# gooey-audio/libgooey

Hardware: NVIDIA B200
Metric: voice-samples/sec (higher is better)
Workload: dtype f32

## Files before the change

### libgooey_b200/csrc/dsp.cuh

```cuda
#pragma once
#include "gmath.cuh"

#ifdef __CUDACC__
#define G_HD __host__ __device__ __forceinline__
#define G_D __device__ __forceinline__
#else
#define G_HD inline
#define G_D inline
#endif

namespace gd {

constexpr float PI_F = 3.14159265358979323846f;

G_HD float clampf(float x, float lo, float hi) { return x < lo ? lo : (x > hi ? hi : x); }
G_HD float denorm(float n, float mn, float mx) { return mn + clampf(n, 0.0f, 1.0f) * (mx - mn); }
G_HD float fract(float x) { return x - truncf(x); }

G_HD float u64_to_f32(uint64_t h) {
#ifdef __CUDA_ARCH__
  return __ull2float_rn(h);
#else
  return (float)h;
#endif
// ... 186 lines not shown
  const uint64_t b = 8ull << 56;
  v3 ^= b; G_SIPROUND v0 ^= b;
  v2 ^= 0xff; G_SIPROUND G_SIPROUND G_SIPROUND
  return v0 ^ v1 ^ v2 ^ v3;
}
G_HD float hash_noise(uint64_t idx) {
  float n = u64_to_f32(siphash13_u64(idx)) / 18446744073709551616.0f;
  return n * 2.0f - 1.0f;
}

constexpr int INV_SQ_N = 1024;
#ifdef __CUDACC__
__constant__ float c_inv_sq[INV_SQ_N];
#endif
template <bool FAST = false> G_HD float osc_sine(float idx, float freq, float sr) {
  const float two_pi = 2.0f * PI_F;
  const float x = idx * freq * two_pi / sr;
  if (FAST) return gm::g_sinf_fast(x);
  return gm::g_sinf(x);
}
G_HD float osc_sine_fast(float idx, float freq, float sr, float rcp_sr) {
  const float two_pi = 2.0f * PI_F;
  return gm::g_sinf_fast(gm::g_div_by(idx * freq * two_pi, sr, rcp_sr));
}
G_HD float inv_sq_odd(int i, float fi) {
#ifdef __CUDA_ARCH__
  return c_inv_sq[i >> 1];
#else
  return 1.0f / (fi * fi);
#endif
}
template <bool FAST> G_HD float tri_partial(float idx, float hf, float sr, float rcp_sr) {
  return FAST ? osc_sine_fast(idx, hf, sr, rcp_sr) : osc_sine<false>(idx, hf, sr);
}
template <bool FAST = false> G_HD float osc_triangle(float idx, float freq, float sr) {
  float output = 0.0f;
  const float nyquist = sr / 2.0f;
  const float rcp_sr = 1.0f / sr;
  const float rcp_nyq = 2.0f * rcp_sr;
  const float lim = 0.7f * nyquist;
  float q = nyquist / freq;
  int max_h = !(q == q) ? 0 : (q >= 2147483648.0f ? 2147483647 : (q <= -2147483648.0f ? (-2147483647 - 1) : (int)q));
  const int cap = (freq > 0.0f && sr > 0.0f) ? (max_h < 2 * INV_SQ_N - 1 ? max_h : 2 * INV_SQ_N - 1) : 0;
  int n1 = 0;
  if (cap >= 1) {
    n1 = ((int)fminf(q * 0.7f, (float)cap) + 1) >> 1;
    while (n1 > 0 && freq * (float)(2 * n1 - 1) > lim) n1--;
    while (2 * n1 + 1 <= cap && !(freq * (float)(2 * n1 + 1) > lim)) n1++;
  }
#ifdef __CUDA_ARCH__
#pragma unroll 4
#endif
  for (int h = 0; h < n1; h++) {
    const int i = 2 * h + 1;
    const float fi = (float)i;
    output += inv_sq_odd(i, fi) * tri_partial<FAST>(idx, freq * fi, sr, rcp_sr);
  }
  int i = 2 * n1 + 1;
  for (; i <= cap; i += 2) {
    const float fi = (float)i;
    const float hf = freq * fi;
    if (hf > nyquist) return output;
    const float ratio = gm::g_div_by(hf, nyquist, rcp_nyq);
    const float t = (ratio - 0.75f) / 0.25f;
    const float taper = ratio > 0.75f ? 1.0f - t * t : 1.0f;
    output += inv_sq_odd(i, fi) * taper * tri_partial<FAST>(idx, hf, sr, rcp_sr);
  }
  for (; i <= max_h; i += 2) {
    float fi = (float)i;
    if (freq * fi > nyquist) break;
    float gain = 1.0f / (fi * fi);
    float hf = freq * fi;
    float taper = 1.0f;
    if (hf > 0.7f * nyquist) {
      float ratio = hf / nyquist;
      if (ratio > 0.75f) { float t = (ratio - 0.75f) / 0.25f; taper = 1.0f - t * t; }
    }
    output += gain * taper * tri_partial<FAST>(idx, hf, sr, rcp_sr);
  }
  return output;
}

constexpr uint64_t XS_SEED = 0x123456789abcdef0ull;
G_HD uint64_t xorshift64s_next(uint64_t& s) {
  uint64_t x = s;
  x ^= x >> 12; x ^= x << 25; x ^= x >> 27;
  s = x;
  return x * 0x2545f4914f6cdd1dull;
}
struct Pink { uint64_t rng; float f0, f1, f2; };
struct PinkCoef { float p0, p1, p2, g0, g1, g2; };
G_HD void pink_reset(Pink& p) { p.rng = XS_SEED; p.f0 = p.f1 = p.f2 = 0.0f; }
G_HD PinkCoef pink_coefs(float sr) {
  const float RP[3] = {0.99765f, 0.96300f, 0.57000f};
  const float RG[3] = {0.0990460f, 0.2965164f, 1.0526913f};
  sr = fmaxf(sr, 1.0f);
  float ratio = 44100.0f / sr;
  float po[3], ga[3];
  for (int i = 0; i < 3; i++) {
    po[i] = gm::g_powf(RP[i], ratio);
    ga[i] = RG[i] * sqrtf((1.0f - po[i] * po[i]) / (1.0f - RP[i] * RP[i]));
  }
  return {po[0], po[1], po[2], ga[0], ga[1], ga[2]};
}
G_HD float pink_tick(Pink& p, const PinkCoef& c) {
  uint64_t h = xorshift64s_next(p.rng);
#ifdef __CUDA_ARCH__
  float w = gm::g_div_by((float)(uint32_t)(h >> 40), 16777215.0f, 0x1.000002p-24f);
#else
  float w = (float)(uint32_t)(h >> 40) / 16777215.0f;
#endif
  w = w * 2.0f - 1.0f;
  p.f0 = c.p0 * p.f0 + c.g0 * w;
  p.f1 = c.p1 * p.f1 + c.g1 * w;
  p.f2 = c.p2 * p.f2 + c.g2 * w;
  float s = 0.0f + p.f0;
  s += p.f1;
  s += p.f2;
  return (s + w * 0.1848f) * 0.11f;
}

struct Tpt { float cutoff, res, g, r, h, ic1, ic2; };
G_HD void tpt_update(Tpt& f, float sr) {
  float cutoff = clampf(f.cutoff, 20.0f, sr * 0.45f);
  float q = fmaxf(f.res, 0.5f);
  float g = gm::g_tanf(PI_F * cutoff / sr);
  float r = 1.0f / q;
  f.g = g; f.r = r; f.h = 1.0f / (1.0f + r * g + g * g);
}
G_HD void tpt_init(Tpt& f, float sr, float cutoff, float res) {
  f.cutoff = clampf(cutoff, 20.0f, 20000.0f); f.res = fmaxf(res, 0.5f); f.ic1 = f.ic2 = 0.0f; tpt_update(f, sr);
}
G_HD void tpt_set(Tpt& f, float sr, float cutoff, float res) {
  float nc = clampf(cutoff, 20.0f, sr * 0.45f);
  float nr = fmaxf(res, 0.5f);
  if (fabsf(nc - f.cutoff) > 0.001f || fabsf(nr - f.res) > 0.001f) { f.cutoff = nc; f.res = nr; tpt_update(f, sr); }
}
G_HD void tpt_process(Tpt& f, float in, float& lo, float& bd, float& hi) {
  float v1 = (f.g * (in - f.ic2) + f.ic1) * f.h;
  float v2 = f.ic2 + f.g * v1;
  f.ic1 = 2.0f * v1 - f.ic1;
  f.ic2 = 2.0f * v2 - f.ic2;
  lo = v2; bd = v1; hi = in - (f.r * v1 + v2);
}
G_HD float svf_pick(float lo, float bd, float hi, uint32_t type) {
  return type == 0 ? lo : (type == 2 ? hi : (type == 3 ? lo + hi : bd));
}
G_HD void rlp_update(Tpt& f, float sr) {
  float s = fmaxf(sr, 1.0f);
  float cutoff = clampf(f.cutoff, 20.0f, s * 0.45f);
  float q = clampf(f.res, 0.5f, 10.0f);
  f.g = gm::g_tanf(PI_F * cutoff / s);
  f.r = 1.0f / q;
  f.h = 1.0f / (1.0f + f.r * f.g + f.g * f.g);
}
G_HD void rlp_init(Tpt& f, float sr, float cutoff, float res) {
  f.cutoff = clampf(cutoff, 20.0f, 20000.0f); f.res = clampf(res, 0.5f, 10.0f); f.ic1 = f.ic2 = 0.0f; rlp_update(f, sr);
}
G_HD void rlp_set(Tpt& f, float sr, float cutoff, float res) {
  cutoff = clampf(cutoff, 20.0f, 20000.0f);
  res = clampf(res, 0.5f, 10.0f);
  if (fabsf(cutoff - f.cutoff) > 0.001f || fabsf(res - f.res) > 0.001f) { f.cutoff = cutoff; f.res = res; rlp_update(f, sr); }
}
G_HD float rlp_process(Tpt& f, float in) {
  float v1 = (f.g * (in - f.ic2) + f.ic1) * f.h;
  float v2 = f.ic2 + f.g * v1;
  f.ic1 = 2.0f * v1 - f.ic1;
  f.ic2 = 2.0f * v2 - f.ic2;
  return fabsf(v2) < 1e-15f ? 0.0f : v2;
// ... 214 lines not shown
```

### libgooey_b200/csrc/wave.cuh

```cuda
#pragma once
#include "kernels.cuh"

namespace gd { namespace wave {

__device__ __forceinline__ float shup(float v, int d) { return __shfl_up_sync(0xffffffffu, v, d); }
__device__ __forceinline__ float shl(float v, int n) { return __shfl_sync(0xffffffffu, v, n); }
__device__ __forceinline__ bool gall(bool p) { return __all_sync(0xffffffffu, p); }
__device__ __forceinline__ unsigned gballot(bool p) { return __ballot_sync(0xffffffffu, p); }
__device__ __forceinline__ void gsync() { __syncwarp(); }

struct Geo1 { float m[5]; float ap; };
struct Geo2 { float a; float m[5]; float ap; };

__device__ __forceinline__ Geo1 make_geo1(float a, int lane) {
  Geo1 g; float p = a, ap = 1.0f; const int e = lane + 1;
#pragma unroll
  for (int i = 0; i < 5; i++) { g.m[i] = lane >= (1 << i) ? p : 0.0f; if (e & (1 << i)) ap *= p; p *= p; }
  if (e & 32) ap *= p;
  g.ap = ap;
  return g;
}
__device__ __forceinline__ Geo2 make_geo2(float a, int lane) {
  Geo2 g; g.a = a; float p = a * a, ap = 1.0f;
#pragma unroll
  for (int i = 0; i < 5; i++) { g.m[i] = lane >= (1 << i) ? p : 0.0f; if (lane & (1 << i)) ap *= p; p *= p; }
  g.ap = ap;
  return g;
}
__device__ __forceinline__ float scan1(float b, const Geo1& g, float y_prev) {
#pragma unroll
  for (int i = 0; i < 5; i++) { float t = shup(b, 1 << i); b = __fmaf_rn(g.m[i], t, b); }
  return __fmaf_rn(g.ap, y_prev, b);
}
__device__ __forceinline__ void scan2(float& b0, float& b1, const Geo2& g, float y_prev, int lane) {
  float B = __fmaf_rn(g.a, b0, b1);
#pragma unroll
  for (int i = 0; i < 5; i++) { float t = shup(B, 1 << i); B = __fmaf_rn(g.m[i], t, B); }
  float yp = shup(B, 1);
  if (lane == 0) yp = 0.0f;
  yp = __fmaf_rn(g.ap, y_prev, yp);
  b0 = __fmaf_rn(g.a, yp, b0);
  b1 = __fmaf_rn(g.a, b0, b1);
}
__device__ __forceinline__ float prev_lane(float v, float carry, int lane) { float t = shup(v, 1); return lane == 0 ? carry : t; }

enum { GT_HB = 0, GT_CLICK = 8, GT_DC = 9, GT_PINK = 10, GT_RING = 13, GT_N1 = 14 };
struct GeoTables {
  float g1[GT_N1][6][32];
  float g2[8][7][32];
};
__device__ __forceinline__ void geo_tables_init(GeoTables& T, const RateCtx& rc, int tid, int nthreads) {
  for (int idx = tid; idx < GT_N1 * 32; idx += nthreads) {
    const int i = idx >> 5, lane = idx & 31;
    float ratio;
    if (i < 8) ratio = -c_hb[i];
    else if (i == GT_CLICK) ratio = 1.0f - rc.click_alpha;
    else if (i == GT_DC) ratio = 0.995f;
    else if (i == GT_PINK) ratio = rc.pink.p0;
    else if (i == GT_PINK + 1) ratio = rc.pink.p1;
    else if (i == GT_PINK + 2) ratio = rc.pink.p2;
    else ratio = 0.999f;
    const Geo1 a = make_geo1(ratio, lane);
#pragma unroll
    for (int k = 0; k < 5; k++) T.g1[i][k][lane] = a.m[k];
    T.g1[i][5][lane] = a.ap;
    if (i < 8) {
      const Geo2 b = make_geo2(ratio, lane);
#pragma unroll
      for (int k = 0; k < 5; k++) T.g2[i][1 + k][lane] = b.m[k];
      T.g2[i][0][lane] = b.a; T.g2[i][6][lane] = b.ap;
    }
  }
}
__device__ __forceinline__ Geo1 load_geo1(const GeoTables& T, int i, int lane) {
  Geo1 g;
#pragma unroll
  for (int k = 0; k < 5; k++) g.m[k] = T.g1[i][k][lane];
  g.ap = T.g1[i][5][lane];
  return g;
}
__device__ __forceinline__ Geo2 load_geo2(const GeoTables& T, int i, int lane) {
  Geo2 g; g.a = T.g2[i][0][lane];
#pragma unroll
  for (int k = 0; k < 5; k++) g.m[k] = T.g2[i][1 + k][lane];
  g.ap = T.g2[i][6][lane];
  return g;
}

__device__ __forceinline__ float ap_sec1(float x, float c, const Geo1& g, float& xs, float& ys, int lane, int last) {
  const float xp = prev_lane(x, xs, lane);
  const float y = scan1(__fmaf_rn(c, x, xp), g, ys);
  xs = shl(x, last); ys = shl(y, last);
  return y;
}
__device__ __forceinline__ void ap_sec2(float& x0, float& x1, float c, const Geo2& g, float& xs, float& ys, int lane, int last) {
  const float xp = prev_lane(x1, xs, lane);
  float b0 = __fmaf_rn(c, x0, xp), b1 = __fmaf_rn(c, x1, x0);
  const float nx = shl(x1, last);
  scan2(b0, b1, g, ys, lane);
  xs = nx; ys = shl(b1, last);
  x0 = b0; x1 = b1;
}
__device__ __forceinline__ void hb_run1(Hb8& s, float& p0, float& p1, const GeoTables& T, int lane, int last) {
#pragma unroll
  for (int i = 0; i < 8; i += 2) {
    p0 = ap_sec1(p0, c_hb[i], load_geo1(T, i, lane), s.x[i], s.y[i], lane, last);
    p1 = ap_sec1(p1, c_hb[i + 1], load_geo1(T, i + 1, lane), s.x[i + 1], s.y[i + 1], lane, last);
  }
}
__device__ __forceinline__ void hb_run2(Hb8& s, float& a0, float& a1, float& b0, float& b1, const GeoTables& T, int lane, int last) {
#pragma unroll
  for (int i = 0; i < 8; i += 2) {
    ap_sec2(a0, a1, c_hb[i], load_geo2(T, i, lane), s.x[i], s.y[i], lane, last);
    ap_sec2(b0, b1, c_hb[i + 1], load_geo2(T, i + 1, lane), s.x[i + 1], s.y[i + 1], lane, last);
  }
}
template <class F> __device__ __forceinline__ float os_scan(Oversamp& o, float in, F f, const GeoTables& T, int lane, int last) {
  if (o.mode == 0) return f(in);
  float s0 = in, s1 = in;
  hb_run1(o.outer_up, s0, s1, T, lane, last);
  if (o.mode == 2) {
    float a = f(s1), b = f(s0);
    hb_run1(o.outer_down, a, b, T, lane, last);
    return 0.5f * (a + b);
  }
  float i00 = s0, i01 = s1, i10 = s0, i11 = s1;
  hb_run2(o.inner_up, i00, i01, i10, i11, T, lane, last);
  float a0 = f(i10), a1 = f(i11), b0 = f(i00), b1 = f(i01);
  hb_run2(o.inner_down, a0, a1, b0, b1, T, lane, last);
  const float d0 = 0.5f * (a0 + b0), d1 = 0.5f * (a1 + b1);
  float a = d1, b = d0;
  hb_run1(o.outer_down, a, b, T, lane, last);
  return 0.5f * (a + b);
}

struct Lin2 {
  float P[5][4];
  float L[4][32];
};
__device__ __forceinline__ void mat_mul(const float* a, const float* b, float* c) {
  c[0] = a[0] * b[0] + a[1] * b[2]; c[1] = a[0] * b[1] + a[1] * b[3];
  c[2] = a[2] * b[0] + a[3] * b[2]; c[3] = a[2] * b[1] + a[3] * b[3];
}
__device__ __forceinline__ void lin2_init(Lin2& S, float m0, float m1, float m2, float m3, int lane) {
  float p[4] = {m0, m1, m2, m3}, acc[4] = {1.0f, 0.0f, 0.0f, 1.0f}, t[4];
  const int e = lane + 1;
#pragma unroll
  for (int i = 0; i < 5; i++) {
    if (lane == 0) { S.P[i][0] = p[0]; S.P[i][1] = p[1]; S.P[i][2] = p[2]; S.P[i][3] = p[3]; }
    if (e & (1 << i)) { mat_mul(p, acc, t); acc[0] = t[0]; acc[1] = t[1]; acc[2] = t[2]; acc[3] = t[3]; }
    mat_mul(p, p, t); p[0] = t[0]; p[1] = t[1]; p[2] = t[2]; p[3] = t[3];
  }
  if (e & 32) { mat_mul(p, acc, t); acc[0] = t[0]; acc[1] = t[1]; acc[2] = t[2]; acc[3] = t[3]; }
  S.L[0][lane] = acc[0]; S.L[1][lane] = acc[1]; S.L[2][lane] = acc[2]; S.L[3][lane] = acc[3];
  gsync();
}
__device__ __forceinline__ void lin2_scan(const Lin2& S, float& f0, float& f1, float s0p, float s1p, int lane) {
#pragma unroll
  for (int i = 0; i < 5; i++) {
    const float t0 = shup(f0, 1 << i), t1 = shup(f1, 1 << i);
    if (lane >= (1 << i)) {
      f0 = __fmaf_rn(S.P[i][0], t0, __fmaf_rn(S.P[i][1], t1, f0));
      f1 = __fmaf_rn(S.P[i][2], t0, __fmaf_rn(S.P[i][3], t1, f1));
    }
  }
  f0 = __fmaf_rn(S.L[0][lane], s0p, __fmaf_rn(S.L[1][lane], s1p, f0));
  f1 = __fmaf_rn(S.L[2][lane], s0p, __fmaf_rn(S.L[3][lane], s1p, f1));
}

struct WaveScratch { Lin2 lin[3]; float stash[8][32]; };


__device__ __forceinline__ float w_tanh(float x) {
  const float ax = fabsf(x);
  const float e = __expf(2.0f * ax);
  const float t = 1.0f - __fdividef(2.0f, e + 1.0f);
  return copysignf(t, x);
}
__device__ __forceinline__ float w_gain_comp(FbShaper& w, float env) {
  const float reference = fmaxf(env, 0.05f);
  const float driven = fmaxf(fabsf(w_tanh(reference * w.drive)), 1e-6f);
  const float comp_no_fb = w_tanh(reference) / driven;
  const float makeup = fbws_makeup(w);
  const float taming = 1.0f / (1.0f + comp_no_fb * w.feedback * 0.25f);
  return fminf(comp_no_fb * taming * makeup, 3.0f);
}
__device__ __forceinline__ float wrap01(float x) { return x < 1.0f ? x : (x < 2.0f ? x - 1.0f : fmodf(x, 1.0f)); }

struct TptLin { float in0, in1; };
__device__ __forceinline__ TptLin tpt_lin_init(Lin2& S, const Tpt& f, int lane) {
  const float g = f.g, h = f.h, gh = g * h, g2h = g * gh;
  lin2_init(S, 2.0f * h - 1.0f, -2.0f * gh, 2.0f * gh, 1.0f - 2.0f * g2h, lane);
  TptLin t; t.in0 = 2.0f * gh; t.in1 = 2.0f * g2h;
  return t;
}
__device__ __forceinline__ void tpt_scan(const Lin2& S, const TptLin& t, Tpt& f, float in, float& ic1_pre, float& ic2_pre, int lane, int last) {
  float s0 = t.in0 * in, s1 = t.in1 * in;
  lin2_scan(S, s0, s1, f.ic1, f.ic2, lane);
  ic1_pre = prev_lane(s0, f.ic1, lane); ic2_pre = prev_lane(s1, f.ic2, lane);
  f.ic1 = shl(s0, last); f.ic2 = shl(s1, last);
}
__device__ __forceinline__ void biquad_lin_init(Lin2& S, const Biquad& b, int lane) { lin2_init(S, -b.a1, -b.a2, 1.0f, 0.0f, lane); }
__device__ __forceinline__ float biquad_scan(const Lin2& S, Biquad& b, float x, int lane, int last) {
  const float xm1 = prev_lane(x, b.x1, lane);
  float xm2 = shup(x, 2);
  xm2 = lane == 0 ? b.x2 : (lane == 1 ? b.x1 : xm2);
  float f0 = b.b0 * x + b.b1 * xm1 + b.b2 * xm2, f1 = 0.0f;
  lin2_scan(S, f0, f1, b.y1, b.y2, lane);
  const float nx1 = shl(x, last), nx2 = shl(xm1, last);
  const float ny1 = shl(f0, last), ny2 = shl(f1, last);
  b.x1 = nx1; b.x2 = nx2; b.y1 = ny1; b.y2 = ny2;
  return fabsf(f0) < 1e-15f ? 0.0f : f0;
}

#define LANE_VAL(v, n) shl((v), (n))
#define STASH_PUT(slot, v) (sc.stash[slot][lane] = (v))
#define STASH_GET(slot, n) (sc.stash[slot][n])

struct KickW {
  using V = KickV;
  struct Span2 { bool noise, shaper, serial; };
  static __device__ __forceinline__ int active_end(const KickV::Run& r) { return r.j_act; }
  static __device__ __forceinline__ void span_setup(KickAud& a, const KickV::Run& r, Span2& w, WaveScratch&, const RateCtx& rc, int) {
    w.noise = r.d.noise_amount > 0.001f;
    a.ws.drive = r.d.drive; a.ws.feedback = r.d.feedback;
    fbws_set_cutoff(a.ws, rc.sr, r.d.fb_cutoff);
    w.shaper = !(a.ws.mix <= 0.0001f || a.ws.drive <= 1.0f);
    w.serial = w.shaper && a.ws.feedback != 0.0f;
    if (w.noise) rlp_set(a.noise_lp, rc.sr, r.d.noise_cut, r.d.noise_res);
  }
  static __device__ __forceinline__ float block(KickAud& a, const KickV::Run& r, const Span2& w, WaveScratch& sc, const GeoTables& T,
                                                const float* p, int, int& nl, const RateCtx& rc, int lane) {
    const int last = nl - 1;
    const float p1 = p[0], raw_click = p[1], ne = p[2], amp = p[3];
    float hp_l = 0.0f, fn_l = 0.0f;
    gsync(); STASH_PUT(0, raw_click); gsync();
#pragma unroll 4
    for (int n = 0; n < nl; n++) {
      const float raw = STASH_GET(0, n);
      const float hp = raw - a.click_hp;
      a.click_hp += rc.click_alpha * hp;
      float fn = 0.0f;
      if (w.noise) fn = rlp_process(a.noise_lp, pink_tick(a.pink, rc.pink));
      if (n == lane) { hp_l = hp; fn_l = fn; }
    }
    const float filt_click = hp_l * (1.0f + 4.0f * 0.1f);
    const float noise_out = w.noise ? fn_l * ne * r.d.noise_amount * 0.5f : 0.0f;
    const float total = p1 + filt_click + noise_out;
    float od = total;
    const bool finite = gall(isfinite(total));
    if (w.serial || (w.shaper && !finite)) {
#pragma unroll 4
      for (int n = 0; n < nl; n++) {
        const float y = fbws_process(a.ws, LANE_VAL(total, n));
        if (n == lane) od = y;
      }
    } else if (w.shaper) {
      FbShaper& ws = a.ws;
      const float fb_in = ws.drive * total + ws.feedback * ws.last_out;
      const float shaped = os_scan(ws.os, fb_in, [](float x) { return w_tanh(x); }, T, lane, last);
      const float rect_l = fabsf(total);
      float env_l = 0.0f;
      gsync(); STASH_PUT(1, rect_l); gsync();
#pragma unroll 4
      for (int n = 0; n < nl; n++) {
        const float rect = STASH_GET(1, n);
        const float coeff = rect > ws.env ? ws.env_att : ws.env_rel;
        ws.env += (1.0f - coeff) * (rect - ws.env);
        if (fabsf(ws.env) < 1e-15f) ws.env = 0.0f;
        if (n == lane) env_l = ws.env;
      }
      const float comp = w_gain_comp(ws, env_l);
      const float compensated = shaped * comp;
      float out_l = 0.0f;
      gsync(); STASH_PUT(2, compensated); gsync();
#pragma unroll 4
      for (int n = 0; n < nl; n++) {
        const float c = STASH_GET(2, n);
        const float out = c - ws.dc_x1 + 0.995f * ws.dc_y1;
        ws.dc_x1 = c;
        ws.dc_y1 = fabsf(out) < 1e-15f ? 0.0f : out;
        ws.filter_state += ws.filter_coeff * (out - ws.filter_state);
        if (fabsf(ws.filter_state) < 1e-15f) ws.filter_state = 0.0f;
        if (n == lane) out_l = out;
      }
      ws.last_out = ws.filter_state;
      od = total * (1.0f - ws.mix) + out_l * ws.mix;
    }
    return od * amp * r.d.va * r.d.volume;
  }
};

struct SnareW {
  using V = SnareV;
  struct Span2 { float comp; bool shaper; };
  static __device__ __forceinline__ int active_end(const SnareV::Run& r) { return r.j_act; }
  static __device__ __forceinline__ void span_setup(SnareAud& a, const SnareV::Run& r, Span2& w, WaveScratch&, const RateCtx& rc, int) {
    chamb_set(a.filt, rc.sr, r.d.cutoff, r.d.res);
    a.ws.drive = r.d.drive;
    w.shaper = !(a.ws.mix <= 0.0001f || a.ws.drive <= 1.0f);
    w.comp = w.shaper ? gm::g_tanhf(0.5f) / gm::g_tanhf(0.5f * a.ws.drive) : 1.0f;
  }
  static __device__ __forceinline__ float block(SnareAud& a, const SnareV::Run& r, const Span2& w, WaveScratch& sc, const GeoTables& T,
                                                const float* p, int, int& nl, const RateCtx&, int lane) {
    const int last = nl - 1;
    const float tonal_out = p[0], raw_noise = p[1], cne = p[2], crack_out = p[3], amp = p[4];
    float low_l = 0.0f, band_l = 0.0f, high_l = 0.0f;
    {
      const float f = a.filt.f, q = a.filt.q;
      float low = a.filt.low, band = a.filt.band;
      gsync(); STASH_PUT(0, raw_noise); gsync();
#pragma unroll 4
      for (int n = 0; n < nl; n++) {
        const float in = STASH_GET(0, n);
        float high = 0.0f;
#pragma unroll
        for (int i = 0; i < 2; i++) { low = low + f * band; high = in - low - q * band; band = f * high + band; }
        if (n == lane) { low_l = low; band_l = band; high_l = high; }
      }
      a.filt.low = low; a.filt.band = band;
    }
    const float filtered = svf_pick(low_l, band_l, high_l, r.d.filter_type);
    const float noise_out = filtered * cne * r.d.noise_mix;
    const float total = tonal_out + noise_out + crack_out;
    float od = total;
    const bool finite = gall(isfinite(total));
    if (!finite) {
#pragma unroll 4
      for (int n = 0; n < nl; n++) {
        const float y = ws_process(a.ws, LANE_VAL(total, n));
        if (n == lane) od = y;
      }
    } else if (w.shaper) {
      const float d = a.ws.drive, comp = w.comp;
      const float sat = os_scan(a.ws.os, total, [d, comp](float x) { return w_tanh(x * d) * comp; }, T, lane, last);
      od = total * (1.0f - a.ws.mix) + sat * a.ws.mix;
    }
    return od * amp * r.d.va * r.d.volume;
  }
};

struct HatW {
  using V = HatV;
  struct Span2 { TptLin svf; };
  static __device__ __forceinline__ int active_end(const HatV::Run&) { return 0x7fffffff; }
  static __device__ __forceinline__ void span_setup(HatAud& a, const HatV::Run& r, Span2& w, WaveScratch& sc, const RateCtx& rc, int lane) {
    hp_set(a.hp1, rc.sr, r.d.pitch_hz, 1.0f);
    biquad_lin_init(sc.lin[0], a.hp1, lane);
    if (r.d.db24) { hp_set(a.hp2, rc.sr, r.d.pitch_hz, 1.0f); biquad_lin_init(sc.lin[1], a.hp2, lane); }
    tpt_set(a.svf, rc.sr, r.d.tone_hz, 0.5f);
    w.svf = tpt_lin_init(sc.lin[2], a.svf, lane);
  }
  static __device__ __forceinline__ float block(HatAud& a, const HatV::Run& r, const Span2& w, WaveScratch& sc, const GeoTables&,
                                                const float* p, int j, int& nl, const RateCtx& rc, int lane) {
    const float sr = rc.sr;
    const float env_l = (j + lane) < r.j_env ? p[0] : r.env_final;
    float es_l = 0.0f;
    int nv = nl;
    gsync(); STASH_PUT(0, env_l); gsync();
    if (j + nl <= r.j_env) {
#pragma unroll 4
      for (int n = 0; n < nl; n++) {
        const float e = STASH_GET(0, n);
        if (e >= a.env_smooth) a.env_smooth = e; else a.env_smooth += rc.asym_down * (e - a.env_smooth);
        if (n == lane) es_l = a.env_smooth;
      }
    } else {
#pragma unroll 4
      for (int n = 0; n < nl; n++) {
        const float e = STASH_GET(0, n);
        if (e >= a.env_smooth) a.env_smooth = e; else a.env_smooth += rc.asym_down * (e - a.env_smooth);
        if (n == lane) es_l = a.env_smooth;
        if ((j + n) >= r.j_env && a.env_smooth < 1e-4f) { nv = n + 1; a.active = 0; break; }
      }
    }
    nl = nv;
    float noise = 0.0f, mph = 0.0f, nph = 0.0f;
    const float inc_mod = fmaxf(r.d.pitch_hz * 0.1f, 0.0f) / sr, inc_main = fmaxf(r.d.pitch_hz, 0.0f) / sr;
    const bool small_inc = inc_main < 1.0f && a.mod_phase < 1.0f && a.main_phase < 1.0f;
    if (!r.d.pink_on && small_inc) {
      uint64_t st_l = 0;
#pragma unroll 4
      for (int n = 0; n < nv; n++) {
        uint64_t x = a.white;
        x ^= x >> 12; x ^= x << 25; x ^= x >> 27;
        a.white = x;
        float pm = a.mod_phase + inc_mod; a.mod_phase = pm < 1.0f ? pm : pm - 1.0f;
        float pn = a.main_phase + inc_main; a.main_phase = pn < 1.0f ? pn : pn - 1.0f;
        if (n == lane) { st_l = x; mph = a.mod_phase; nph = a.main_phase; }
      }
      const float u = u64_to_f32(st_l * 0x2545f4914f6cdd1dull) / 18446744073709551616.0f;
      noise = (u * 2.0f) - 1.0f;
    } else {
#pragma unroll 4
      for (int n = 0; n < nv; n++) {
        float x;
        if (r.d.pink_on) x = pink_tick(a.pink, rc.pink);
        else { float u = u64_to_f32(xorshift64s_next(a.white)) / 18446744073709551616.0f; x = (u * 2.0f) - 1.0f; }
        a.mod_phase = wrap01(a.mod_phase + inc_mod);
        a.main_phase = wrap01(a.main_phase + inc_main);
        if (n == lane) { noise = x; mph = a.mod_phase; nph = a.main_phase; }
      }
    }
    float ph = mph + noise * 0.25f; ph -= floorf(ph);
    const float mod_out = gm::g_sinf(2.0f * PI_F * ph);
    ph = nph + mod_out * 0.75f; ph -= floorf(ph);
    const float main_out = gm::g_sinf(2.0f * PI_F * ph);
    const int last = nv - 1;
    float filtered = biquad_scan(sc.lin[0], a.hp1, main_out, lane, last);
    if (r.d.db24) filtered = biquad_scan(sc.lin[1], a.hp2, filtered, lane, last) * 0.8f;
    const float out = filtered * es_l * r.d.vel035 * 0.35f;
    float ic1p, ic2p;
    tpt_scan(sc.lin[2], w.svf, a.svf, out, ic1p, ic2p, lane, last);
    const float v1 = (a.svf.g * (out - ic2p) + ic1p) * a.svf.h;
    const float v2 = ic2p + a.svf.g * v1;
    const float hi = out - (a.svf.r * v1 + v2);
    return hi * r.d.volume;
  }
};

struct TomW {
  using V = TomV;
  struct Span2 { int dummy; };
  static __device__ __forceinline__ int active_end(const TomV::Run&) { return 0x7fffffff; }
  static __device__ __forceinline__ void span_setup(TomAud&, const TomV::Run&, Span2&, WaveScratch&, const RateCtx&, int) {}
  static __device__ __forceinline__ float generic(TomAud& a, const TomV::Run& r, WaveScratch& sc, float env_l, float noise_l, float rnd_l,
                                                  int j, int& nl, const RateCtx& rc, int lane) {
    float y_l = 0.0f;
    int nv = nl;
    gsync(); STASH_PUT(0, env_l); STASH_PUT(1, noise_l); STASH_PUT(2, rnd_l); gsync();
#pragma unroll 2
    for (int n = 0; n < nl; n++) {
      TomFront f; f.env = STASH_GET(0, n); f.noise = STASH_GET(1, n); f.rnd = STASH_GET(2, n);
      const float y = tom_back(a, r.d, f, (j + n) >= r.j_env, rc);
      if (n == lane) y_l = y;
      if (!a.active) { nv = n + 1; break; }
    }
    nl = nv;
    return y_l;
  }
  static __device__ __forceinline__ float membrane(TomAud& a, WaveScratch& sc, float mi_l, int nv, int lane) {
    const float u1 = shup(mi_l, 1), u2 = shup(mi_l, 2);
    gsync();
#pragma unroll
    for (int f = 0; f < 5; f++) {
      const Biquad& m = a.mem[f];
      const float xm1 = lane == 0 ? m.x1 : u1, xm2 = lane == 0 ? m.x2 : (lane == 1 ? m.x1 : u2);
      sc.stash[f][lane] = m.b0 * mi_l + m.b1 * xm1 + m.b2 * xm2;
    }
    const float nx1 = shl(mi_l, nv - 1), nx2 = nv >= 2 ? shl(mi_l, nv - 2) : a.mem[0].x1;
#pragma unroll
    for (int f = 0; f < 5; f++) { a.mem[f].x2 = nv >= 2 ? nx2 : a.mem[f].x1; a.mem[f].x1 = nx1; }
    float a1 = a.mem[4].a1, a2 = a.mem[4].a2, y1 = a.mem[4].y1, y2 = a.mem[4].y2;
#pragma unroll
    for (int f = 0; f < 4; f++) if (lane == f) { a1 = a.mem[f].a1; a2 = a.mem[f].a2; y1 = a.mem[f].y1; y2 = a.mem[f].y2; }
    const int row = lane < 5 ? lane : 4;
    gsync();
#pragma unroll 4
    for (int n = 0; n < nv; n++) {
      const float out = sc.stash[row][n] - a1 * y1 - a2 * y2;
      y2 = y1; y1 = out;
      if (lane < 5) sc.stash[row][n] = fabsf(out) < 1e-15f ? 0.0f : out;
    }
    gsync();
    float acc = 0.0f;
#pragma unroll
    for (int i = 0; i < 5; i++) acc += sc.stash[i][lane];
#pragma unroll
    for (int i = 0; i < 5; i++) { a.mem[i].y1 = shl(y1, i); a.mem[i].y2 = shl(y2, i); }
    return w_tanh(acc);
  }
  static __device__ __forceinline__ float block(TomAud& a, const TomV::Run& r, const Span2&, WaveScratch& sc, const GeoTables&,
                                                const float* p, int j, int& nl, const RateCtx& rc, int lane) {
    const TomDer& d = r.d;
    const float sr = rc.sr;
    const float env_l = (j + lane) < r.j_env ? p[0] : r.env_final;
    const float noise_l = p[1], rnd_l = p[2];
    const bool complete_l = (j + lane) >= r.j_env;
    const unsigned valid = nl >= 32 ? 0xffffffffu : ((1u << nl) - 1u);
    const unsigned le = (2u << lane) - 1u;
    const float eb = env_l * d.bend_scaled;
    const float raw_freq = d.base_frequency * (1.0f + eb * eb);
    const unsigned m_att = gballot(env_l > 0.9f) & valid;
    const bool past_l = a.past_attack || (m_att & le) != 0u;
    const unsigned m_done = gballot(complete_l || (past_l && raw_freq < 20.0f)) & valid;
    const int first_done = a.main_done ? 0 : (m_done ? __ffs(m_done) - 1 : 32);
    const bool merged = a.tri_phase == a.main_sine_phase && a.tri_phase == a.mtri_phase && a.tri_phase == a.gated_sine_phase;
    if (first_done == 0) {
      if (d.membrane > 0.0f && j >= r.j_env) {
        a.main_done = 1;
        const float eb0 = r.env_final * d.bend_scaled;
        bp_set(a.bp, sr, fmaxf(fmaxf(d.base_frequency * (1.0f + eb0 * eb0), 40.0f), 20.0f), d.fq, 1.1f);
        const float clipped = membrane(a, sc, 0.0f, nl, lane);
        gsync(); STASH_PUT(5, fabsf(clipped) * 0.001f); gsync();
        float lev_l = 0.0f;
        int nv = nl;
        for (int n = 0; n < nl; n++) {
          if (!(a.ring_level > 0.0001f)) { nv = n; a.active = 0; break; }
          a.ring_level = a.ring_level * 0.999f + STASH_GET(5, n);
          if (n == lane) lev_l = a.ring_level;
        }
        nl = nv;
        const float fd = lev_l >= 0.005f ? 1.0f : (lev_l <= 0.0001f ? 0.0f : (lev_l - 0.0001f) / (0.005f - 0.0001f));
        return clipped * d.mm * fd * 0.7f * d.vol;
      }
      if (!(d.membrane > 0.0f) && !(a.ring_level > 0.0001f)) {
        a.main_done = 1; a.active = 0; if (m_att & 1u) a.past_attack = 1;
        nl = 0;
        return 0.0f;
      }
      return generic(a, r, sc, env_l, noise_l, rnd_l, j, nl, rc, lane);
    }
    if (!merged) return generic(a, r, sc, env_l, noise_l, rnd_l, j, nl, rc, lane);
    const int nv = first_done < nl ? first_done : nl;
    a.past_attack = a.past_attack || (m_att & (nv >= 32 ? 0xffffffffu : ((1u << nv) - 1u))) != 0u;
    nl = nv;
    const float fade = (past_l && raw_freq < 40.0f) ? (raw_freq - 20.0f) / (40.0f - 20.0f) : 1.0f;
    const float mf_l = fmaxf(raw_freq, 40.0f);
    float click = 0.0f;
    if (a.click_playing) {
      const uint32_t idx = a.click_pos + (uint32_t)lane;
      if (idx < 64u) click = c_tom_impulse[idx];
      a.click_pos = min(64u, a.click_pos + (uint32_t)nv);
      if (a.click_pos >= 64u) a.click_playing = 0;
    }
    const float ff_l = fmaxf(mf_l, 20.0f);
    const float inc_fixed = 190.0f / sr, inc_rand = d.rand_freq / sr;
    gsync(); STASH_PUT(0, mf_l / sr); STASH_PUT(1, rnd_l); STASH_PUT(2, ff_l); gsync();
    unsigned mask = 0u;
    {
      float ph = a.tri_phase, fx = a.fixed_sine_phase, rph = a.rand_phase, rcu = a.rand_current, rtg = a.rand_target, lf = a.bp.last_freq;
      bool qg_ok = fabsf(d.fq - a.bp.last_q) < 0.001f && fabsf(1.1f - a.bp.last_gain) < 0.001f;
#pragma unroll 4
      for (int n = 0; n < nv; n++) {
        const float inc = STASH_GET(0, n), rnd = STASH_GET(1, n), ffn = STASH_GET(2, n);
        sc.stash[3][n] = ph; sc.stash[4][n] = fx;
        ph += inc; if (ph >= 1.0f) ph -= 1.0f;
        fx += inc_fixed; if (fx >= 1.0f) fx -= 1.0f;
        const float prev = rph;
        rph += inc_rand; if (rph >= 1.0f) rph -= 1.0f;
        const bool wrap = rph < prev;
        rcu = wrap ? rtg : rcu; rtg = wrap ? rnd : rtg;
        sc.stash[5][n] = rcu + (rtg - rcu) * rph;
        const bool upd = !(fabsf(ffn - lf) < 0.01f && qg_ok);
        lf = upd ? ffn : lf; qg_ok = qg_ok || upd;
        mask |= upd ? (1u << n) : 0u;
      }
      a.tri_phase = a.main_sine_phase = a.mtri_phase = a.gated_sine_phase = ph;
      a.fixed_sine_phase = fx; a.rand_phase = rph; a.rand_current = rcu; a.rand_target = rtg;
      a.bp.last_freq = lf;
      if (mask) { a.bp.last_q = d.fq; a.bp.last_gain = 1.1f; }
    }
    gsync();
    const float tp = sc.stash[3][lane], fsp = sc.stash[4][lane], rand_value = sc.stash[5][lane];
    const float click_out = click * 1.1f;
    const float tri_out = a.tri_enabled ? tri_wave(tp) * 0.5f : 0.0f;
    const float us = unit_sine(tp);
    const float main_sine = us * 0.5f;
    const float mtri = tri_wave(tp) * 0.5f;
    const float fixed_sine = unit_sine(fsp) * 0.5f;
    const float noise = noise_l * 0.2f;
    const float noise_combined = (noise + rand_value) * 0.4f;
    const float gated = d.tone < 99.0f ? us * 0.2f : 0.0f;
    const float ch1 = main_sine * fixed_sine, ch2 = mtri + noise_combined, ch3 = noise_combined + gated;
    const float morph_out = ch1 * d.w1 + ch2 * d.w2 + ch3 * d.w3;
    const float x = click_out + tri_out + morph_out;
    float b0 = a.bp.b0, b1 = a.bp.b1, b2 = a.bp.b2, a1 = a.bp.a1, a2 = a.bp.a2;
    if (mask) {
      Biquad spec;
      bp_compute(spec, sr, ff_l, d.fq, 1.1f);
      const unsigned m = mask & le;
      const int src = m ? 31 - __clz(m) : 0;
      const float sb0 = shl(spec.b0, src), sb1 = shl(spec.b1, src), sb2 = shl(spec.b2, src), sa1 = shl(spec.a1, src), sa2 = shl(spec.a2, src);
      if (m) { b0 = sb0; b1 = sb1; b2 = sb2; a1 = sa1; a2 = sa2; }
    }
    float xm1 = shup(x, 1), xm2 = shup(x, 2);
    if (lane == 0) { xm1 = a.bp.x1; xm2 = a.bp.x2; } else if (lane == 1) xm2 = a.bp.x1;
    const float ffwd = b0 * x + b1 * xm1 + b2 * xm2;
    gsync(); STASH_PUT(0, ffwd); STASH_PUT(1, a1); STASH_PUT(2, a2); gsync();
    {
      const int last = nv - 1;
      a.bp.b0 = shl(b0, last); a.bp.b1 = shl(b1, last); a.bp.b2 = shl(b2, last); a.bp.a1 = shl(a1, last); a.bp.a2 = shl(a2, last);
      a.bp.x1 = shl(x, last); a.bp.x2 = shl(xm1, last);
    }
    {
      float y1 = a.bp.y1, y2 = a.bp.y2;
#pragma unroll 4
      for (int n = 0; n < nv; n++) {
        const float out = STASH_GET(0, n) - STASH_GET(1, n) * y1 - STASH_GET(2, n) * y2;
        y2 = y1; y1 = out;
        sc.stash[3][n] = fabsf(out) < 1e-15f ? 0.0f : out;
      }
      a.bp.y1 = y1; a.bp.y2 = y2;
    }
    gsync();
    const float filtered = sc.stash[3][lane];
    float mem_out = 0.0f;
    if (d.membrane > 0.0f) {
      mem_out = membrane(a, sc, filtered * env_l, nv, lane);
      gsync(); STASH_PUT(5, fabsf(mem_out) * 0.001f); gsync();
#pragma unroll 4
      for (int n = 0; n < nv; n++) a.ring_level = a.ring_level * 0.999f + STASH_GET(5, n);
    }
    const float dry_gain = 1.0f - d.mm;
    const float dry = filtered * env_l;
    const float fs = dry * dry_gain + mem_out * d.mm;
    return fs * fade * 0.7f * d.vol;
  }
};

template <class W>
__global__ void __launch_bounds__(32, 1) wave_kernel(const VoiceLaunch L) {
  using V = typename W::V; using Span = typename V::Span; using Aud = typename V::Aud;
  constexpr int WC = sizeof(typename V::Ctl) / 4;
  __shared__ GeoTables T;
  __shared__ WaveScratch sc;
  const int lane = threadIdx.x & 31;
  geo_tables_init(T, L.rc, threadIdx.x, 32);
  __syncthreads();
  const int v = blockIdx.x;
  const bool alive = v < L.n && L.mode[v] == 0;
  const int sv = alive ? (L.slots ? (int)L.slots[v] : v) : 0;
  Aud a;
  const Span* spans = nullptr;
  uint32_t ns = 0, cur = 0xffffffffu;
  typename V::Run run;
  typename W::Span2 w2;
  bool ready = false;
  int next_j0 = 0x7fffffff;
  float* out = nullptr;
  const float* planes = nullptr;
  if (alive) {
    load_words(a, L.state, sv, L.n_pad, WC);
    spans = reinterpret_cast<const Span*>(L.spans) + L.span_off[v];
    ns = L.n_spans[v];
    cur = L.span_cursor[v];
    if (cur != 0xffffffffu) V::span_resume(spans[cur], run);
    next_j0 = cur + 1u < ns ? spans[cur + 1u].j0 : 0x7fffffff;
    const long long row = L.rows ? (long long)L.rows[v] : (long long)(L.row0 + v);
    out = L.out + row * L.stride;
    planes = L.planes + (size_t)v * L.pitch;
  }
  const int c1 = L.chunk0 + min(L.chunk_frames, L.frames - L.chunk0);
  int j = L.chunk0;
  while (alive && j < c1) {
    while (j == next_j0) {
      cur += 1u;
      V::span_begin(a, spans[cur], run, L.rc.sr);
      ready = false;
      next_j0 = cur + 1u < ns ? spans[cur + 1u].j0 : 0x7fffffff;
    }
    const int span_end = min(next_j0, c1);
    const int act_end = min(span_end, W::active_end(run));
    if (cur == 0xffffffffu || !V::is_active(a, run, j) || j >= act_end) {
      for (int k = j + lane; k < span_end; k += 32) out[k] = 0.0f;
      j = span_end;
      continue;
    }
    if (!ready) { gsync(); W::span_setup(a, run, w2, sc, L.rc, lane); ready = true; }
    int nl = min(32, act_end - j);
    float p[V::NPL];
    const int jj = j + min(lane, nl - 1);
#pragma unroll
    for (int q = 0; q < V::NPL; q++) p[q] = planes[(size_t)q * L.plane_stride + (jj - L.chunk0)];
    const float y = W::block(a, run, w2, sc, T, p, j, nl, L.rc, lane);
    if (lane < nl) out[j + lane] = y;
    j += nl;
  }
  if (alive && lane == 0) {
    store_words(a, L.state, sv, L.n_pad, WC);
    L.span_cursor[v] = cur;
  }
}

#undef LANE_VAL
} }
```

Baseline: 8.889 billion.

## Parallelize xorshift noise across lanes with GF(2) jump tables and sample-and-hold ballot

Takes xorshift64 state generation out of the serial per-sample loop. Each lane now gets its own RNG state from a precomputed shared-memory jump table, a 32-step jump expressed as a GF(2) matrix with 4-bit lookup, and does the hash and pink-input scaling in parallel. Only the cheap pink IIR recurrence stays serial. Tom's sample-and-hold random value is likewise computed after the loop using a ballot over phase wraps instead of being carried serially. This shortens the serial dependency chain at the cost of extra shared memory, table initialization per block, and a fallback serial walk when a block is not a full 32 samples.

```diff
diff --git a/libgooey_b200/csrc/dsp.cuh b/libgooey_b200/csrc/dsp.cuh
--- a/libgooey_b200/csrc/dsp.cuh
+++ b/libgooey_b200/csrc/dsp.cuh
@@ -292,9 +292,9 @@
 }
 
 constexpr uint64_t XS_SEED = 0x123456789abcdef0ull;
+G_HD uint64_t xs_step(uint64_t x) { x ^= x >> 12; x ^= x << 25; x ^= x >> 27; return x; }
 G_HD uint64_t xorshift64s_next(uint64_t& s) {
-  uint64_t x = s;
-  x ^= x >> 12; x ^= x << 25; x ^= x >> 27;
+  const uint64_t x = xs_step(s);
   s = x;
   return x * 0x2545f4914f6cdd1dull;
 }
diff --git a/libgooey_b200/csrc/noise_jump.cuh b/libgooey_b200/csrc/noise_jump.cuh
--- /dev/null
+++ b/libgooey_b200/csrc/noise_jump.cuh
@@ -0,0 +1,68 @@
+#pragma once
+#include "dsp.cuh"
+
+namespace gd {
+
+constexpr int XS_JUMP = 32;
+struct XsJump { uint64_t t[16][16]; };
+G_HD void xs_jump_init(XsJump& J, int tid, int nthreads) {
+  for (int b = tid; b < 64; b += nthreads) {
+    uint64_t x = 1ull << b;
+    for (int k = 0; k < XS_JUMP; k++) x = xs_step(x);
+    J.t[b >> 2][1 << (b & 3)] = x;
+  }
+#ifdef __CUDA_ARCH__
+  __syncthreads();
+#endif
+  for (int idx = tid; idx < 256; idx += nthreads) {
+    const int i = idx >> 4, v = idx & 15;
+    if (v & (v - 1) || v == 0) {
+      uint64_t r = 0;
+      for (int bit = 0; bit < 4; bit++) if (v >> bit & 1) r ^= J.t[i][1 << bit];
+      J.t[i][v] = r;
+    }
+  }
+}
+G_HD uint64_t xs_jump(const XsJump& J, uint64_t s) {
+  uint64_t r = 0;
+#pragma unroll
+  for (int i = 0; i < 16; i++) r ^= J.t[i][(s >> (4 * i)) & 15u];
+  return r;
+}
+
+struct PinkIn { float gw0, gw1, gw2, wk; };
+G_HD PinkIn pink_in(uint64_t state, const PinkCoef& c) {
+  const uint64_t h = state * 0x2545f4914f6cdd1dull;
+#ifdef __CUDA_ARCH__
+  float w = gm::g_div_by((float)(uint32_t)(h >> 40), 16777215.0f, 0x1.000002p-24f);
+#else
+  float w = (float)(uint32_t)(h >> 40) / 16777215.0f;
+#endif
+  w = w * 2.0f - 1.0f;
+  PinkIn q; q.gw0 = c.g0 * w; q.gw1 = c.g1 * w; q.gw2 = c.g2 * w; q.wk = w * 0.1848f;
+  return q;
+}
+G_HD float pink_replay(Pink& p, const PinkCoef& c, float gw0, float gw1, float gw2, float wk) {
+  p.f0 = c.p0 * p.f0 + gw0;
+  p.f1 = c.p1 * p.f1 + gw1;
+  p.f2 = c.p2 * p.f2 + gw2;
+  float s = 0.0f + p.f0;
+  s += p.f1;
+  s += p.f2;
+  return (s + wk) * 0.11f;
+}
+
+G_HD int hi_bit(unsigned m) {
+#ifdef __CUDA_ARCH__
+  return 31 - __clz(m);
+#else
+  return 31 - __builtin_clz(m);
+#endif
+}
+G_HD void snh_sources(unsigned wraps, int& tg, int& cu) {
+  tg = wraps ? hi_bit(wraps) : -1;
+  const unsigned rest = wraps ? wraps & ~(1u << tg) : 0u;
+  cu = rest ? hi_bit(rest) : -1;
+}
+
+}
diff --git a/libgooey_b200/csrc/wave.cuh b/libgooey_b200/csrc/wave.cuh
--- a/libgooey_b200/csrc/wave.cuh
+++ b/libgooey_b200/csrc/wave.cuh
@@ -1,5 +1,6 @@
 #pragma once
 #include "kernels.cuh"
+#include "noise_jump.cuh"
 
 namespace gd { namespace wave {
 
@@ -87,6 +88,31 @@
   return g;
 }
 
+struct XsLane { uint64_t s; bool ok; };
+__device__ __forceinline__ uint64_t xs_lane_state(const XsLane& xl, uint64_t s0, int n, int lane) {
+  if (xl.ok) return xl.s;
+  uint64_t x = s0, st = 0;
+#pragma unroll 4
+  for (int k = 0; k < n; k++) { x = xs_step(x); if (k == lane) st = x; }
+  return st;
+}
+__device__ __forceinline__ uint64_t xs_lane_advance(XsLane& xl, const XsJump& J, uint64_t st, int n) {
+  xl.ok = n == XS_JUMP;
+  if (xl.ok) xl.s = xs_jump(J, st);
+  return __shfl_sync(0xffffffffu, st, n - 1);
+}
+
+__device__ __forceinline__ float snh_block(float rph_l, float rph_prev, float rnd_l, int nv, int lane, float& cur, float& tgt) {
+  const unsigned wraps = gballot(rph_l < rph_prev) & (nv >= 32 ? 0xffffffffu : ((1u << nv) - 1u));
+  int tg, cu;
+  snh_sources(wraps & ((2u << lane) - 1u), tg, cu);
+  const float s_tg = shl(rnd_l, tg < 0 ? 0 : tg), s_cu = shl(rnd_l, cu < 0 ? 0 : cu);
+  const float rtg = tg < 0 ? tgt : s_tg;
+  const float rcu = cu >= 0 ? s_cu : (tg >= 0 ? tgt : cur);
+  cur = shl(rcu, nv - 1); tgt = shl(rtg, nv - 1);
+  return rcu + (rtg - rcu) * rph_l;
+}
+
 __device__ __forceinline__ float ap_sec1(float x, float c, const Geo1& g, float& xs, float& ys, int lane, int last) {
   const float xp = prev_lane(x, xs, lane);
   const float y = scan1(__fmaf_rn(c, x, xp), g, ys);
@@ -219,6 +245,7 @@
 
 struct KickW {
   using V = KickV;
+  static constexpr bool XS = true;
   struct Span2 { bool noise, shaper, serial; };
   static __device__ __forceinline__ int active_end(const KickV::Run& r) { return r.j_act; }
   static __device__ __forceinline__ void span_setup(KickAud& a, const KickV::Run& r, Span2& w, WaveScratch&, const RateCtx& rc, int) {
@@ -230,20 +257,28 @@
     if (w.noise) rlp_set(a.noise_lp, rc.sr, r.d.noise_cut, r.d.noise_res);
   }
   static __device__ __forceinline__ float block(KickAud& a, const KickV::Run& r, const Span2& w, WaveScratch& sc, const GeoTables& T,
-                                                const float* p, int, int& nl, const RateCtx& rc, int lane) {
+                                                const XsJump& J, XsLane& xl, const float* p, int, int& nl, const RateCtx& rc, int lane) {
     const int last = nl - 1;
     const float p1 = p[0], raw_click = p[1], ne = p[2], amp = p[3];
     float hp_l = 0.0f, fn_l = 0.0f;
-    gsync(); STASH_PUT(0, raw_click); gsync();
+    uint64_t st_l = 0;
+    gsync(); STASH_PUT(0, raw_click);
+    if (w.noise) {
+      st_l = xs_lane_state(xl, a.pink.rng, nl, lane);
+      const PinkIn q = pink_in(st_l, rc.pink);
+      STASH_PUT(1, q.gw0); STASH_PUT(2, q.gw1); STASH_PUT(3, q.gw2); STASH_PUT(4, q.wk);
+    }
+    gsync();
 #pragma unroll 4
     for (int n = 0; n < nl; n++) {
       const float raw = STASH_GET(0, n);
       const float hp = raw - a.click_hp;
       a.click_hp += rc.click_alpha * hp;
       float fn = 0.0f;
-      if (w.noise) fn = rlp_process(a.noise_lp, pink_tick(a.pink, rc.pink));
+      if (w.noise) fn = rlp_process(a.noise_lp, pink_replay(a.pink, rc.pink, STASH_GET(1, n), STASH_GET(2, n), STASH_GET(3, n), STASH_GET(4, n)));
       if (n == lane) { hp_l = hp; fn_l = fn; }
     }
+    if (w.noise) a.pink.rng = xs_lane_advance(xl, J, st_l, nl);
     const float filt_click = hp_l * (1.0f + 4.0f * 0.1f);
     const float noise_out = w.noise ? fn_l * ne * r.d.noise_amount * 0.5f : 0.0f;
     const float total = p1 + filt_click + noise_out;
@@ -293,6 +328,7 @@
 
 struct SnareW {
   using V = SnareV;
+  static constexpr bool XS = false;
   struct Span2 { float comp; bool shaper; };
   static __device__ __forceinline__ int active_end(const SnareV::Run& r) { return r.j_act; }
   static __device__ __forceinline__ void span_setup(SnareAud& a, const SnareV::Run& r, Span2& w, WaveScratch&, const RateCtx& rc, int) {
@@ -302,7 +338,7 @@
     w.comp = w.shaper ? gm::g_tanhf(0.5f) / gm::g_tanhf(0.5f * a.ws.drive) : 1.0f;
   }
   static __device__ __forceinline__ float block(SnareAud& a, const SnareV::Run& r, const Span2& w, WaveScratch& sc, const GeoTables& T,
-                                                const float* p, int, int& nl, const RateCtx&, int lane) {
+                                                const XsJump&, XsLane&, const float* p, int, int& nl, const RateCtx&, int lane) {
     const int last = nl - 1;
     const float tonal_out = p[0], raw_noise = p[1], cne = p[2], crack_out = p[3], amp = p[4];
     float low_l = 0.0f, band_l = 0.0f, high_l = 0.0f;
@@ -342,6 +378,7 @@
 
 struct HatW {
   using V = HatV;
+  static constexpr bool XS = true;
   struct Span2 { TptLin svf; };
   static __device__ __forceinline__ int active_end(const HatV::Run&) { return 0x7fffffff; }
   static __device__ __forceinline__ void span_setup(HatAud& a, const HatV::Run& r, Span2& w, WaveScratch& sc, const RateCtx& rc, int lane) {
@@ -352,7 +389,7 @@
     w.svf = tpt_lin_init(sc.lin[2], a.svf, lane);
   }
   static __device__ __forceinline__ float block(HatAud& a, const HatV::Run& r, const Span2& w, WaveScratch& sc, const GeoTables&,
-                                                const float* p, int j, int& nl, const RateCtx& rc, int lane) {
+                                                const XsJump& J, XsLane& xl, const float* p, int j, int& nl, const RateCtx& rc, int lane) {
     const float sr = rc.sr;
     const float env_l = (j + lane) < r.j_env ? p[0] : r.env_final;
     float es_l = 0.0f;
@@ -376,32 +413,36 @@
     }
     nl = nv;
     float noise = 0.0f, mph = 0.0f, nph = 0.0f;
+    const bool pink = r.d.pink_on;
+    const uint64_t st_l = xs_lane_state(xl, pink ? a.pink.rng : a.white, nv, lane);
+    if (pink) {
+      const PinkIn q = pink_in(st_l, rc.pink);
+      gsync(); STASH_PUT(1, q.gw0); STASH_PUT(2, q.gw1); STASH_PUT(3, q.gw2); STASH_PUT(4, q.wk); gsync();
+    } else {
+      const float u = u64_to_f32(st_l * 0x2545f4914f6cdd1dull) / 18446744073709551616.0f;
+      noise = (u * 2.0f) - 1.0f;
+    }
     const float inc_mod = fmaxf(r.d.pitch_hz * 0.1f, 0.0f) / sr, inc_main = fmaxf(r.d.pitch_hz, 0.0f) / sr;
     const bool small_inc = inc_main < 1.0f && a.mod_phase < 1.0f && a.main_phase < 1.0f;
-    if (!r.d.pink_on && small_inc) {
-      uint64_t st_l = 0;
+    if (!pink && small_inc) {
 #pragma unroll 4
       for (int n = 0; n < nv; n++) {
-        uint64_t x = a.white;
-        x ^= x >> 12; x ^= x << 25; x ^= x >> 27;
-        a.white = x;
         float pm = a.mod_phase + inc_mod; a.mod_phase = pm < 1.0f ? pm : pm - 1.0f;
         float pn = a.main_phase + inc_main; a.main_phase = pn < 1.0f ? pn : pn - 1.0f;
-        if (n == lane) { st_l = x; mph = a.mod_phase; nph = a.main_phase; }
-      }
-      const float u = u64_to_f32(st_l * 0x2545f4914f6cdd1dull) / 18446744073709551616.0f;
-      noise = (u * 2.0f) - 1.0f;
+        if (n == lane) { mph = a.mod_phase; nph = a.main_phase; }
+      }
     } else {
 #pragma unroll 4
       for (int n = 0; n < nv; n++) {
-        float x;
-        if (r.d.pink_on) x = pink_tick(a.pink, rc.pink);
-        else { float u = u64_to_f32(xorshift64s_next(a.white)) / 18446744073709551616.0f; x = (u * 2.0f) - 1.0f; }
+        float x = 0.0f;
+        if (pink) x = pink_replay(a.pink, rc.pink, STASH_GET(1, n), STASH_GET(2, n), STASH_GET(3, n), STASH_GET(4, n));
         a.mod_phase = wrap01(a.mod_phase + inc_mod);
         a.main_phase = wrap01(a.main_phase + inc_main);
-        if (n == lane) { noise = x; mph = a.mod_phase; nph = a.main_phase; }
-      }
-    }
+        if (n == lane) { if (pink) noise = x; mph = a.mod_phase; nph = a.main_phase; }
+      }
+    }
+    const uint64_t st_end = xs_lane_advance(xl, J, st_l, nv);
+    if (pink) a.pink.rng = st_end; else a.white = st_end;
     float ph = mph + noise * 0.25f; ph -= floorf(ph);
     const float mod_out = gm::g_sinf(2.0f * PI_F * ph);
     ph = nph + mod_out * 0.75f; ph -= floorf(ph);
@@ -421,6 +462,7 @@
 
 struct TomW {
   using V = TomV;
+  static constexpr bool XS = false;
   struct Span2 { int dummy; };
   static __device__ __forceinline__ int active_end(const TomV::Run&) { return 0x7fffffff; }
   static __device__ __forceinline__ void span_setup(TomAud&, const TomV::Run&, Span2&, WaveScratch&, const RateCtx&, int) {}
@@ -471,7 +513,7 @@
     return w_tanh(acc);
   }
   static __device__ __forceinline__ float block(TomAud& a, const TomV::Run& r, const Span2&, WaveScratch& sc, const GeoTables&,
-                                                const float* p, int j, int& nl, const RateCtx& rc, int lane) {
+                                                const XsJump&, XsLane&, const float* p, int j, int& nl, const RateCtx& rc, int lane) {
     const TomDer& d = r.d;
     const float sr = rc.sr;
     const float env_l = (j + lane) < r.j_env ? p[0] : r.env_final;
@@ -526,33 +568,32 @@
     }
     const float ff_l = fmaxf(mf_l, 20.0f);
     const float inc_fixed = 190.0f / sr, inc_rand = d.rand_freq / sr;
-    gsync(); STASH_PUT(0, mf_l / sr); STASH_PUT(1, rnd_l); STASH_PUT(2, ff_l); gsync();
+    const float rph0 = a.rand_phase;
+    gsync(); STASH_PUT(0, mf_l / sr); STASH_PUT(2, ff_l); gsync();
     unsigned mask = 0u;
     {
-      float ph = a.tri_phase, fx = a.fixed_sine_phase, rph = a.rand_phase, rcu = a.rand_current, rtg = a.rand_target, lf = a.bp.last_freq;
+      float ph = a.tri_phase, fx = a.fixed_sine_phase, rph = rph0, lf = a.bp.last_freq;
       bool qg_ok = fabsf(d.fq - a.bp.last_q) < 0.001f && fabsf(1.1f - a.bp.last_gain) < 0.001f;
 #pragma unroll 4
       for (int n = 0; n < nv; n++) {
-        const float inc = STASH_GET(0, n), rnd = STASH_GET(1, n), ffn = STASH_GET(2, n);
+        const float inc = STASH_GET(0, n), ffn = STASH_GET(2, n);
         sc.stash[3][n] = ph; sc.stash[4][n] = fx;
         ph += inc; if (ph >= 1.0f) ph -= 1.0f;
         fx += inc_fixed; if (fx >= 1.0f) fx -= 1.0f;
-        const float prev = rph;
         rph += inc_rand; if (rph >= 1.0f) rph -= 1.0f;
-        const bool wrap = rph < prev;
-        rcu = wrap ? rtg : rcu; rtg = wrap ? rnd : rtg;
-        sc.stash[5][n] = rcu + (rtg - rcu) * rph;
+        sc.stash[5][n] = rph;
         const bool upd = !(fabsf(ffn - lf) < 0.01f && qg_ok);
         lf = upd ? ffn : lf; qg_ok = qg_ok || upd;
         mask |= upd ? (1u << n) : 0u;
       }
       a.tri_phase = a.main_sine_phase = a.mtri_phase = a.gated_sine_phase = ph;
-      a.fixed_sine_phase = fx; a.rand_phase = rph; a.rand_current = rcu; a.rand_target = rtg;
+      a.fixed_sine_phase = fx; a.rand_phase = rph;
       a.bp.last_freq = lf;
       if (mask) { a.bp.last_q = d.fq; a.bp.last_gain = 1.1f; }
     }
     gsync();
-    const float tp = sc.stash[3][lane], fsp = sc.stash[4][lane], rand_value = sc.stash[5][lane];
+    const float tp = sc.stash[3][lane], fsp = sc.stash[4][lane], rph_l = sc.stash[5][lane];
+    const float rand_value = snh_block(rph_l, lane == 0 ? rph0 : sc.stash[5][lane > 0 ? lane - 1 : 0], rnd_l, nv, lane, a.rand_current, a.rand_target);
     const float click_out = click * 1.1f;
     const float tri_out = a.tri_enabled ? tri_wave(tp) * 0.5f : 0.0f;
     const float us = unit_sine(tp);
@@ -614,10 +655,13 @@
   using V = typename W::V; using Span = typename V::Span; using Aud = typename V::Aud;
   constexpr int WC = sizeof(typename V::Ctl) / 4;
   __shared__ GeoTables T;
+  __shared__ XsJump J;
   __shared__ WaveScratch sc;
   const int lane = threadIdx.x & 31;
   geo_tables_init(T, L.rc, threadIdx.x, 32);
+  if constexpr (W::XS) xs_jump_init(J, threadIdx.x, 32);
   __syncthreads();
+  XsLane xl; xl.s = 0; xl.ok = false;
   const int v = blockIdx.x;
   const bool alive = v < L.n && L.mode[v] == 0;
   const int sv = alive ? (L.slots ? (int)L.slots[v] : v) : 0;
@@ -657,13 +701,13 @@
       j = span_end;
       continue;
     }
-    if (!ready) { gsync(); W::span_setup(a, run, w2, sc, L.rc, lane); ready = true; }
+    if (!ready) { gsync(); W::span_setup(a, run, w2, sc, L.rc, lane); ready = true; xl.ok = false; }
     int nl = min(32, act_end - j);
     float p[V::NPL];
     const int jj = j + min(lane, nl - 1);
 #pragma unroll
     for (int q = 0; q < V::NPL; q++) p[q] = planes[(size_t)q * L.plane_stride + (jj - L.chunk0)];
-    const float y = W::block(a, run, w2, sc, T, p, j, nl, L.rc, lane);
+    const float y = W::block(a, run, w2, sc, T, J, xl, p, j, nl, L.rc, lane);
     if (lane < nl) out[j + lane] = y;
     j += nl;
   }
```

Result: faster. 9.454 billion, median of 6 (+6.4%).
